# randyjhc/vit-colmap

Measured on AMD Instinct MI355X. Metric: images/sec extracted + pair-matches/sec (N×D brute-force NN), higher is better.
Workload: dtype bf16 (ViT) / u8+i32 (matcher); 1 GPU; configs[1]+configs[2]: DINOv2 ViT-S/14 extract of 50 640x480 images (512 keypoints, 384-D uint8 descriptors) then exhaustive mutual-NN + ratio matching of all pairs among the extracted images; images_total=50, images_rank0=50, num_keypoints=512, descriptor_dim=384, parallelism=images+pairs sharded x1

## Files before the change

### include/vitcolmap_hip.h

```cpp
#ifndef VITCOLMAP_HIP_H_
#define VITCOLMAP_HIP_H_

#include <stddef.h>
#include <stdint.h>

#ifdef __cplusplus
extern "C" {
#endif

#define VC_ABI_VERSION 1

#define VC_OK 0
#define VC_ERR_INVALID_ARG (-1)
#define VC_ERR_UNSUPPORTED (-2)
#define VC_ERR_LAUNCH (-3)
#define VC_ERR_WORKSPACE (-4)

#define VC_MAX_KEYPOINTS 2048
#define VC_MAX_DESC_DIM 1024
#define VC_MAX_NEIGHBOURS 64

typedef void* vc_stream_t;

int vc_abi_version(void);
// ... 134 lines not shown
#define VC_LAYOUT_NCHW 0
#define VC_LAYOUT_PATCHES 1
#define VC_LAYOUT_PATCHES_PAD 2
#define VC_PATCH_K_PADDED 640

int vc_preprocess_u8(const uint8_t* images_bgr, int n_images, int h, int w, int out_h, int out_w,
                     int out_dtype, int layout, void* out, uint8_t* resized_bgr_or_null,
                     vc_stream_t stream);

int vc_add_layernorm_bf16(const void* x, const void* residual_or_null, const void* gamma,
                          const void* beta, float eps, int rows, int C, void* sum_out_or_null,
                          void* y_out, vc_stream_t stream);

int vc_layernorm_drop_first_bf16(const void* x, const void* gamma, const void* beta, float eps, int n_groups,
                                 int group_rows, int C, void* y_out, vc_stream_t stream);

int vc_attention_bf16(const void* qkv, int batch, int n_tokens, int n_heads, int head_dim, int q_prescaled,
                      void* out, vc_stream_t stream);

#define VC_EPI_BIAS 0
#define VC_EPI_GELU 1
#define VC_EPI_RESIDUAL 2
#define VC_EPI_SWIGLU 4
int vc_linear_bf16(const void* x, const void* weight, const void* bias, const void* residual_or_null,
                   void* out, int rows, int n_out, int k_in, int epilogue, vc_stream_t stream);

int vc_conv_taps_bf16(void* x, const void* weight, const void* bias, void* out, int batch, int height, int width, int c_in,
                      int n_out, int kh, int kw, int dy0, int dx0, int out_parity, int epilogue, vc_stream_t stream);

size_t vc_linear_xs_weight_bytes(int n_out, int k_in);
// ... 57 lines not shown
```

### vit_colmap_amd/_lib.py

```python
import ctypes
import os
from ctypes import POINTER, c_char_p, c_double, c_float, c_int, c_int32, c_size_t, c_uint8, c_uint32, c_void_p

_HERE = os.path.dirname(os.path.abspath(__file__))
LIB_PATH = os.environ.get("VITCOLMAP_HIP_LIB") or os.path.join(_HERE, "libvitcolmap_hip.so")

VC_OK = 0
ABI_VERSION = 1
VC_MAX_KEYPOINTS = 2048
VC_MAX_DESC_DIM = 1024
VC_MAX_NEIGHBOURS = 64
VC_BA_MAX_CAMS = 512
VC_BA_MAX_GROUPS = 8
VC_ERR_INVALID_ARG, VC_ERR_UNSUPPORTED, VC_ERR_LAUNCH, VC_ERR_WORKSPACE = -1, -2, -3, -4


class HipLibraryError(RuntimeError):
    pass


_u8p, _i32p, _u32p, _f32p = POINTER(c_uint8), POINTER(c_int32), POINTER(c_uint32), POINTER(ctypes.c_float)

SIGNATURES = {
    "vc_abi_version": (c_int, []),
# ... 42 lines not shown
    "vc_score_map": (c_int, [c_void_p, c_int, c_int, c_int, c_int, c_void_p, c_void_p]),
    "vc_select_keypoints": (c_int, [c_void_p, c_int, c_int, c_int, c_int, c_int, c_float, c_int, c_void_p,
                                    c_void_p, c_void_p, c_void_p, c_void_p, c_void_p, c_void_p]),
    "vc_describe": (c_int, [c_void_p, c_int, c_int, c_int, c_int, c_int, c_void_p, c_void_p, c_int, c_void_p,
                            c_int, c_int, c_int, c_int, c_int, c_void_p, c_void_p, c_void_p, c_void_p]),
    "vc_describe_at": (c_int, [c_void_p, c_int, c_int, c_int, c_int, c_int, c_void_p, c_void_p, c_int, c_void_p, c_int, c_int,
                               c_int, c_int, c_int, c_int, c_void_p, c_void_p, c_void_p]),
    "vc_quantize_u8": (c_int, [c_void_p, c_void_p, c_size_t, c_void_p]),
    "vc_heatmap_workspace_bytes": (c_size_t, [c_int, c_int, c_int, c_int]),
    "vc_heatmap_keypoints": (c_int, [c_void_p, c_void_p, ctypes.c_longlong, ctypes.c_longlong, ctypes.c_longlong, c_int, c_int,
                                     c_int, c_int, c_int, c_float, c_int, c_float, c_float, c_float, c_float, c_void_p,
                                     c_void_p, c_void_p, c_void_p, c_void_p]),
    "vc_add_layernorm_bf16": (c_int, [c_void_p, c_void_p, c_void_p, c_void_p, c_float, c_int, c_int, c_void_p,
                                      c_void_p, c_void_p]),
    "vc_layernorm_drop_first_bf16": (c_int, [c_void_p, c_void_p, c_void_p, c_float, c_int, c_int, c_int, c_void_p, c_void_p]),
    "vc_attention_bf16": (c_int, [c_void_p, c_int, c_int, c_int, c_int, c_int, c_void_p, c_void_p]),
    "vc_linear_bf16": (c_int, [c_void_p, c_void_p, c_void_p, c_void_p, c_void_p, c_int, c_int, c_int, c_int, c_void_p]),
    "vc_conv_taps_bf16": (c_int, [c_void_p, c_void_p, c_void_p, c_void_p] + [c_int] * 11 + [c_void_p]),
    "vc_linear_xs_weight_bytes": (c_size_t, [c_int, c_int]),
    "vc_linear_xs_prepare": (c_int, [c_void_p, c_void_p, c_void_p, c_void_p, c_int, c_int, c_void_p, c_void_p, c_void_p]),
    "vc_linear_xs_bf16": (c_int, [c_void_p, c_void_p, c_void_p, c_void_p, c_void_p, c_int, c_int, c_int, c_int, c_int,
                                  c_float, c_void_p, c_void_p]),
    "vc_gelu_table_bytes": (c_size_t, []),
    "vc_gelu_table_bf16": (c_int, [c_void_p, c_void_p]),
    "vc_patch_embed_bf16": (c_int, [c_void_p, c_void_p, c_void_p, c_void_p, c_void_p, c_int, c_int, c_int, c_int, c_void_p]),
    "vc_mlp_weight_bytes": (c_size_t, [c_int, c_int]),
    "vc_mlp_prepare": (c_int, [c_void_p, c_void_p, c_void_p, c_void_p, c_void_p, c_void_p, c_int, c_int, c_void_p, c_void_p,
                               c_void_p, c_void_p]),
    "vc_mlp_bf16": (c_int, [c_void_p, c_void_p, c_void_p, c_void_p, c_void_p, c_int, c_int, c_int, c_float, c_void_p]),
    "vc_preprocess_u8": (c_int, [c_void_p, c_int, c_int, c_int, c_int, c_int, c_int, c_int, c_void_p, c_void_p,
# ... 102 lines not shown
```

### vit_colmap_amd/csrc/select.hip

```cpp
#include <hip/hip_runtime.h>
#include <stdint.h>

#include "../../include/vitcolmap_hip.h"
#include "common.h"
#include "device.h"

namespace {

constexpr int kMaxCells = 16384;
constexpr int kMaxCandidates = 4096;
constexpr int kSelThreads = 512;

template <typename T>
__device__ inline float load_token(const T* p, int i);
template <>
__device__ inline float load_token<float>(const float* p, int i) { return p[i]; }
template <>
__device__ inline float load_token<uint16_t>(const uint16_t* p, int i) { return vc::bf16_to_f32(p[i]); }

__device__ inline float wave_sum(float v) {
#pragma unroll
  for (int o = 32; o > 0; o >>= 1) v += __shfl_xor(v, o);
  return v;
}

template <typename T>
__global__ __launch_bounds__(256) void structure_tensor_kernel(const T* __restrict__ tokens, int H, int W, int C,
                                                               float* __restrict__ st, bool vec_ok) {
  const int lane = threadIdx.x & 63;
  const int cells = H * W;
  const int cell = blockIdx.x * 4 + (threadIdx.x >> 6);
  const int img = blockIdx.y;
  if (cell >= cells) return;
  const int y = cell / W, x = cell - y * W;
  const T* f = tokens + ((size_t)img * cells + cell) * C;
  const bool has_r = x + 1 < W, has_d = y + 1 < H;
  const T* fr = f + C;
  const T* fd = f + (size_t)W * C;
  float sxx = 0.f, syy = 0.f, sxy = 0.f, sm = 0.f;
  if (vec_ok) {
    typedef uint32_t v4u __attribute__((ext_vector_type(4)));
    constexpr int NQ = (int)sizeof(T) / 2;
    for (int c0 = lane * 8; c0 < C; c0 += 64 * 8) {
      const v4u zero = {0u, 0u, 0u, 0u};
      v4u qv[NQ], qr[NQ], qd[NQ];
#pragma unroll
      for (int q = 0; q < NQ; ++q) {
        qv[q] = *((const v4u*)(f + c0) + q);
        qr[q] = has_r ? *((const v4u*)(fr + c0) + q) : zero;
        qd[q] = has_d ? *((const v4u*)(fd + c0) + q) : zero;
      }
#pragma unroll
      for (int j = 0; j < 8; ++j) {
        float v, r, d;
        if (sizeof(T) == 4) {
          v = __uint_as_float(qv[j >> 2][j & 3]); r = __uint_as_float(qr[j >> 2][j & 3]); d = __uint_as_float(qd[j >> 2][j & 3]);
        } else {
          const int sh = (j & 1) * 16;
          v = __uint_as_float(((qv[0][j >> 1] >> sh) & 0xffffu) << 16);
          r = __uint_as_float(((qr[0][j >> 1] >> sh) & 0xffffu) << 16);
          d = __uint_as_float(((qd[0][j >> 1] >> sh) & 0xffffu) << 16);
        }
        const float gx = has_r ? r - v : 0.f;
        const float gy = has_d ? d - v : 0.f;
        sxx += gx * gx;
        syy += gy * gy;
        sxy += gx * gy;
        sm += v;
      }
    }
  } else {
    for (int c = lane; c < C; c += 64) {
      const float v = load_token<T>(f, c);
      const float gx = has_r ? load_token<T>(fr, c) - v : 0.f;
      const float gy = has_d ? load_token<T>(fd, c) - v : 0.f;
      sxx += gx * gx;
      syy += gy * gy;
      sxy += gx * gy;
      sm += v;
    }
  }
  sxx = wave_sum(sxx); syy = wave_sum(syy); sxy = wave_sum(sxy); sm = wave_sum(sm);
  if (lane == 0) {
    float* o = st + (size_t)img * 4 * cells + cell;
    const float inv = (float)C;
    o[0] = sxx / inv;
    o[cells] = syy / inv;
    o[2 * cells] = sxy / inv;
    o[3 * cells] = sm / inv;
  }
}

struct Taps {
  float w[11];
  int k;
};

__device__ inline float zero_pad(const float* m, int H, int W, int y, int x) {
  return (y >= 0 && y < H && x >= 0 && x < W) ? m[y * W + x] : 0.f;
}

__device__ inline float smooth(const float* m, int H, int W, int y, int x, const Taps& t) {
  const int r = t.k / 2;
  float acc = 0.f;
  for (int dy = 0; dy < t.k; ++dy)
// ... 90 lines not shown

__device__ inline bool before(float sa, int pa, float sb, int pb) { return sa > sb || (sa == sb && pa < pb); }

__global__ __launch_bounds__(kSelThreads) void select_kernel(const float* __restrict__ score_g, int H, int W,
                                                             int target, int bin, int nms_reach, int nms_d2_max, int kmax,
                                                             int32_t* __restrict__ out_yx,
                                                             float* __restrict__ out_score,
                                                             int32_t* __restrict__ out_count,
                                                             int32_t* __restrict__ dbg_cand_yx,
                                                             float* __restrict__ dbg_cand_score,
                                                             int32_t* __restrict__ dbg_cand_count) {
  extern __shared__ __attribute__((aligned(16))) float lds[];
  const int cells = H * W;
  const int tid = threadIdx.x, nt = blockDim.x;
  const int img = blockIdx.x;
  float* score = lds;
  int* cand_cell = (int*)(lds + cells);
  float* cand_score = (float*)(cand_cell + kMaxCandidates);
  int* tmp_cell = (int*)(cand_score + kMaxCandidates);
  float* tmp_score = (float*)(tmp_cell + kMaxCandidates);
  int* state = (int*)(tmp_score + kMaxCandidates);
  int* cell_rank = state + kMaxCandidates;
  __shared__ int s_wave_tot[kSelThreads / 64];

  for (int i = tid; i < cells; i += nt) score[i] = score_g[(size_t)img * cells + i];
  __syncthreads();

  const int nbh = max(1, H / bin), nbw = max(1, W / bin);
  const int per_bin = max(1, target / (nbh * nbw));
  const int bh = min(bin, H), bw = min(bin, W), n = bh * bw;
  const int k = min(per_bin, n);
  const int K_bins = nbh * nbw * k;
  for (int idx = tid; idx < nbh * nbw * n; idx += nt) {
    const int b = idx / n, e = idx - b * n;
    const int bi = b / nbw, bj = b - bi * nbw;
    const int y0 = bi * bin, x0 = bj * bin;
    const int ey = e / bw, ex = e - ey * bw;
    const float s = score[(y0 + ey) * W + x0 + ex];
    int rank = 0;
    for (int oy = 0; oy < bh; ++oy)
      for (int ox = 0; ox < bw; ++ox)
        rank += before(score[(y0 + oy) * W + x0 + ox], oy * bw + ox, s, e) ? 1 : 0;
    if (rank < k) {
      cand_cell[b * k + rank] = (y0 + ey) * W + x0 + ex;
      cand_score[b * k + rank] = s;
    }
  }
  int K = K_bins;
  __syncthreads();

  int run_len = k, n_runs = nbh * nbw;
  auto merged_rank = [&](int e) {
    const float s = cand_score[e];
    const int mine = e / run_len;
    int rank = e - mine * run_len;
    for (int q = 0; q < n_runs; ++q) {
      if (q == mine) continue;
      int lo = 0, hi = run_len;
      while (lo < hi) {
// ... 334 lines not shown
```

### vit_colmap_amd/csrc/vit_ops.hip

```cpp
#include <hip/hip_runtime.h>
#include <stdint.h>

#include "../../include/vitcolmap_hip.h"
#include "common.h"
#include "device.h"

namespace {

typedef uint16_t bf16_t;
constexpr int kMaxChunksPerLane = 4;

__device__ inline float wsum(float v) {
#pragma unroll
  for (int o = 32; o > 0; o >>= 1) v += __shfl_xor(v, o);
  return v;
}

struct alignas(16) Vec8 { bf16_t e[8]; };

template <bool HAS_RES, bool WRITE_SUM>
__global__ __launch_bounds__(256) void add_layernorm_kernel(const bf16_t* __restrict__ x,
                                                            const bf16_t* __restrict__ res,
                                                            const bf16_t* __restrict__ gamma,
                                                            const bf16_t* __restrict__ beta, float eps,
                                                            int rows, int C, bf16_t* __restrict__ sum_out,
                                                            bf16_t* __restrict__ y_out, int drop_group) {
  const int lane = threadIdx.x & 63;
  const int row = blockIdx.x * 4 + (threadIdx.x >> 6);
  if (row >= rows) return;
  const int nchunk = C >> 3;
  const size_t base = (size_t)row * C;
  size_t ybase = base;
  if (drop_group > 0) {
// ... 12 lines not shown
      if (HAS_RES) b = *(const Vec8*)(res + base + ch * 8);
      Vec8 o;
#pragma unroll
      for (int i = 0; i < 8; ++i) {
        float t = vc::bf16_to_f32(a.e[i]);
        if (HAS_RES) {
          o.e[i] = vc::f32_to_bf16(t + vc::bf16_to_f32(b.e[i]));
          t = vc::bf16_to_f32(o.e[i]);
        }
        v[k][i] = t;
        s += t;
      }
      if (HAS_RES && WRITE_SUM) *(Vec8*)(sum_out + base + ch * 8) = o;
    }
  }
  const float mean = wsum(s) / (float)C;
  float q = 0.f;
#pragma unroll
  for (int k = 0; k < kMaxChunksPerLane; ++k) {
    if (lane + 64 * k < nchunk) {
#pragma unroll
      for (int i = 0; i < 8; ++i) { const float d = v[k][i] - mean; q += d * d; }
    }
  }
  const float rstd = rsqrtf(wsum(q) / (float)C + eps);
#pragma unroll
  for (int k = 0; k < kMaxChunksPerLane; ++k) {
    const int ch = lane + 64 * k;
    if (ch < nchunk) {
      const Vec8 g = *(const Vec8*)(gamma + ch * 8);
      const Vec8 bb = *(const Vec8*)(beta + ch * 8);
      Vec8 o;
#pragma unroll
      for (int i = 0; i < 8; ++i) o.e[i] = vc::f32_to_bf16((v[k][i] - mean) * rstd * vc::bf16_to_f32(g.e[i]) + vc::bf16_to_f32(bb.e[i]));
      *(Vec8*)(y_out + ybase + ch * 8) = o;
    }
  }
}

}

extern "C" {

static int add_layernorm_launch(const void* x, const void* residual_or_null, const void* gamma, const void* beta, float eps,
                                int rows, int C, void* sum_out_or_null, void* y_out, int drop_group, vc_stream_t stream);

int vc_add_layernorm_bf16(const void* x, const void* residual_or_null, const void* gamma, const void* beta,
                          float eps, int rows, int C, void* sum_out_or_null, void* y_out, vc_stream_t stream) {
  return add_layernorm_launch(x, residual_or_null, gamma, beta, eps, rows, C, sum_out_or_null, y_out, 0, stream);
}

int vc_layernorm_drop_first_bf16(const void* x, const void* gamma, const void* beta, float eps, int n_groups, int group_rows,
                                 int C, void* y_out, vc_stream_t stream) {
  if (n_groups < 0 || group_rows < 2) return VC_ERR_INVALID_ARG;
  return add_layernorm_launch(x, nullptr, gamma, beta, eps, n_groups * group_rows, C, nullptr, y_out, group_rows, stream);
}

static int add_layernorm_launch(const void* x, const void* residual_or_null, const void* gamma, const void* beta, float eps,
                                int rows, int C, void* sum_out_or_null, void* y_out, int drop_group, vc_stream_t stream) {
  if (!x || !gamma || !beta || !y_out || rows < 0 || C <= 0) return VC_ERR_INVALID_ARG;
  if (C % 8 != 0 || C > 64 * kMaxChunksPerLane * 8) return VC_ERR_UNSUPPORTED;
  if ((((uintptr_t)x) | ((uintptr_t)y_out) | ((uintptr_t)gamma) | ((uintptr_t)beta) |
       ((uintptr_t)residual_or_null) | ((uintptr_t)sum_out_or_null)) % 16 != 0)
    return VC_ERR_INVALID_ARG;
  if (rows == 0) return VC_OK;
  const dim3 grid((rows + 3) / 4), block(256);
  hipStream_t s = (hipStream_t)stream;
  const bf16_t *px = (const bf16_t*)x, *pr = (const bf16_t*)residual_or_null, *pg = (const bf16_t*)gamma,
               *pb = (const bf16_t*)beta;
  bf16_t *ps = (bf16_t*)sum_out_or_null, *py = (bf16_t*)y_out;
  if (!pr)
    hipLaunchKernelGGL((add_layernorm_kernel<false, false>), grid, block, 0, s, px, pr, pg, pb, eps, rows, C, ps, py, drop_group);
  else if (ps)
    hipLaunchKernelGGL((add_layernorm_kernel<true, true>), grid, block, 0, s, px, pr, pg, pb, eps, rows, C, ps, py, drop_group);
  else
    hipLaunchKernelGGL((add_layernorm_kernel<true, false>), grid, block, 0, s, px, pr, pg, pb, eps, rows, C, ps, py, drop_group);
  return vc::check_launch();
}

// ... 2 lines not shown
```

### vit_colmap_amd/features/hip_select.py

```python
import torch

from .. import _lib

METHODS = {"harris": 0, "dog": 1, "combined": 2}


def _dtype_code(t):
    if t.dtype == torch.float32:
        return 0
    if t.dtype == torch.bfloat16:
        return 1
    raise _lib.HipLibraryError(f"tokens must be float32 or bfloat16, got {t.dtype}")


def _check_tokens(tokens, H, W):
    if not tokens.is_cuda:
        raise _lib.HipLibraryError("tokens must live on the GPU (no CPU fallback)")
    assert tokens.dim() == 3 and tokens.is_contiguous() and tokens.shape[1] == H * W, tokens.shape


def structure_tensor(tokens: torch.Tensor, H: int, W: int) -> torch.Tensor:
    _check_tokens(tokens, H, W)
    lib = _lib.load()
    B, _, C = tokens.shape
# ... 75 lines not shown
                                  _lib.ptr(projection), dd, int(feature_wh[0]), int(feature_wh[1]), int(original_wh[0]),
                                  int(original_wh[1]), 1 if rootsift else 0, _lib.ptr(f32), _lib.ptr(u8), _lib.stream_ptr()),
               "vc_describe_at")
    return (u8, f32) if want_f32 else u8


def quantize_u8(x: torch.Tensor) -> torch.Tensor:
    assert x.is_cuda and x.dtype == torch.float32 and x.is_contiguous()
    lib = _lib.load()
    out = torch.empty(x.shape, dtype=torch.uint8, device=x.device)
    _lib.check(lib.vc_quantize_u8(_lib.ptr(x), _lib.ptr(out), x.numel(), _lib.stream_ptr()), "vc_quantize_u8")
    return out


def dense_to_sparse(tokens, H, W, original_wh, resized_wh, num_keypoints, method="harris", projection=None,
                    bin_size=16, nms_radius=1.5, want_f32=False):
    st = structure_tensor(tokens, H, W)
    score = score_map(st, H, W, method)
    yx, sc, cnt = select_keypoints(score, num_keypoints, bin_size, nms_radius)
    out = describe(tokens, H, W, yx, cnt, resized_wh, original_wh, projection, want_f32)
    res = dict(keypoints=out[0], desc_u8=out[1], count=cnt, yx=yx, scores=sc, score=score)
    if want_f32:
        res["desc_f32"] = out[2]
    return res


def heatmap_workspace_bytes(n_images: int, H: int, W: int, kmax: int) -> int:
    return _lib.load().vc_heatmap_workspace_bytes(n_images, H, W, kmax)


def heatmap_keypoints(kp_map: torch.Tensor, desc_map: torch.Tensor, num_keypoints: int, score_threshold: float,
                      nms_radius: int, original_wh, resized_wh):
# ... 24 lines not shown
```

### vit_colmap_amd/features/vit_extractor.py

```python
import os
from pathlib import Path
from typing import Optional

import numpy as np
import torch

from .. import _lib
from ..utils import image_io
from ..vit import build_dinov2, load_dinov2_weights
from . import hip_preprocess, hip_select
from .base_extractor import BaseExtractor, default_camera_params, extract_to_database, host_rows, list_images

PATCH = 14


class ViTExtractor(BaseExtractor):
    camera_params_for = staticmethod(default_camera_params)
    camera_per_image = False

    def __init__(
        self,
        weights_path: str | None = None,
        model_name: str = "dinov2_vitb14",
        num_keypoints: int = 2048,
# ... 79 lines not shown
            files = list_images(Path(image_dir))
            first = image_io.imread(files[0]) if files else None
            if first is not None:
                self._run_batch([first])
        have = vd.broadcast_array(np.array([self.descriptor_projection is not None], np.int32), 0, str(self.device))
        if int(have[0]):
            p = vd.broadcast_array(self.descriptor_projection.cpu().numpy() if rank == 0 else None, 0, str(self.device))
            self.set_projection(p)

    def _require_gpu(self):
        if self.device.type != "cuda":
            raise _lib.HipLibraryError(
                "ViTExtractor needs an MI355X: the selection / descriptor path is HIP-only (no CPU fallback)")

    @torch.inference_mode()
    def _tokens(self, images_bgr: torch.Tensor):
        B, h, w, _ = images_bgr.shape
        hp, wp = h // PATCH, w // PATCH
        if self.model.accepts_padded_patches:
            patches = hip_preprocess.preprocess(images_bgr, out_dtype=self.dtype, layout="patches_pad")
            return self.model.forward_patch_tokens(patches, hp, wp).contiguous(), hp, wp
        patches = hip_preprocess.preprocess(images_bgr, out_dtype=self.dtype, layout="patches")
        if self.tune_gemm:
            import torch.cuda.tunable as tunable

            was = tunable.is_enabled()
            tunable.enable(True)
            try:
                tokens = self.model.forward_patch_tokens(patches, hp, wp).contiguous()
            finally:
                tunable.enable(was)
        else:
            tokens = self.model.forward_patch_tokens(patches, hp, wp).contiguous()
        return tokens, hp, wp

    @torch.inference_mode()
# ... 16 lines not shown
            g = torch.Generator(device="cpu").manual_seed(self.seed)
            p = torch.randn(C, self.descriptor_dim, generator=g, dtype=torch.float32) / np.sqrt(C)
            self.descriptor_projection = p.to(self.device)
            print(f"Initialized random projection (insufficient samples): {C} -> {self.descriptor_dim}")

    batch_shards = None

    def _shard_bounds(self, B, pipelined=False):
        k = self.batch_shards if self.batch_shards is not None else int(os.environ.get("VITCOLMAP_VIT_SHARDS", "1" if pipelined else "2"))
        if k <= 1 or B < 8 * k or not getattr(self.model, "_hip", None):
            return None
        return [B * i // k for i in range(k + 1)]

    def _extract_one(self, images_bgr, hw):
        h, w, h_new, w_new = hw
        tokens, hp, wp = self._tokens(images_bgr)
        self._ensure_projection(tokens, hp, wp, (w, h), (w_new, h_new))
        proj = self.descriptor_projection if tokens.shape[-1] > self.descriptor_dim else None
        return hip_select.dense_to_sparse(tokens, hp, wp, (w, h), (w_new, h_new), self.num_keypoints,
                                          self.detection_method, proj)

    @torch.inference_mode()
    def extract_device(self, images_bgr: torch.Tensor, input_ready=None):
        self._require_gpu()
        B, h, w, _ = images_bgr.shape
        hw = (h, w, (h // PATCH) * PATCH, (w // PATCH) * PATCH)
        bounds = self._shard_bounds(B, pipelined=input_ready is not None)
        needs_fit = self.model.arch.dim > self.descriptor_dim and self.descriptor_projection is None
        if needs_fit or (bounds is None and (input_ready is None or not getattr(self.model, "_hip", None))):
            return self._extract_one(images_bgr, hw)
        if bounds is None:
            bounds = [0, B]
        dev = images_bgr.device
        n_sh = len(bounds) - 1
        n_streams = max(n_sh, int(os.environ.get("VITCOLMAP_VIT_STREAMS", "2")))
# ... 30 lines not shown
            cur.wait_event(done)
            for t in part.values():
                t.record_stream(cur)
        if len(parts) == 1:
            return parts[0]
        return {k: torch.cat([p[k] for p in parts]) for k in parts[0]}

    @torch.inference_mode()
    def _run_batch(self, images_bgr_np):
        self._require_gpu()
        h, w = images_bgr_np[0].shape[:2]
        h_new, w_new = (h // PATCH) * PATCH, (w // PATCH) * PATCH
        if h_new == 0 or w_new == 0:
            raise ValueError(f"image {w}x{h} is smaller than one 14x14 patch")
        batch = torch.from_numpy(np.ascontiguousarray(np.stack(images_bgr_np))).to(self.device, non_blocking=True)
        tokens, hp, wp = self._tokens(batch)
        self._ensure_projection(tokens, hp, wp, (w, h), (w_new, h_new))
        proj = self.descriptor_projection if tokens.shape[-1] > self.descriptor_dim else None
        res = hip_select.dense_to_sparse(tokens, hp, wp, (w, h), (w_new, h_new), self.num_keypoints,
                                         self.detection_method, proj)
        return host_rows(res["count"], res["keypoints"], res["desc_u8"])

    def _staging(self, slot, shape):
        bufs = self.__dict__.setdefault("_pinned_in", {})
        n = int(np.prod(shape))
        if slot not in bufs or bufs[slot].numel() < n:
            bufs[slot] = torch.empty(n, dtype=torch.uint8, pin_memory=True)
        return bufs[slot][:n].view(shape)

    @torch.inference_mode()
    def _launch_batch(self, images_bgr_np):
        self._require_gpu()
        h, w = images_bgr_np[0].shape[:2]
        if (h // PATCH) * PATCH == 0 or (w // PATCH) * PATCH == 0:
            raise ValueError(f"image {w}x{h} is smaller than one 14x14 patch")
# ... 43 lines not shown
```

### vit_colmap_amd/vit/dinov2.py

```python
import math
from dataclasses import dataclass

import torch
import torch.nn as nn
import torch.nn.functional as F

PATCH = 14


@dataclass(frozen=True)
class Arch:
    dim: int
    depth: int
    heads: int
    ffn: str = "mlp"
    registers: int = 0
    img_size: int = 518


DINOV2_ARCHS = {
    "dinov2_vits14": Arch(384, 12, 6),
    "dinov2_vitb14": Arch(768, 12, 12),
    "dinov2_vitl14": Arch(1024, 24, 16),
    "dinov2_vitg14": Arch(1536, 40, 24, ffn="swiglu"),
# ... 173 lines not shown
            if self.accepts_padded_patches:
                self._padded_pos(hp, wp, device)
            elif self.pos_embed.device == device:
                self.interpolated_pos_embed(hp, wp)
            if device.type != "cuda":
                return None
            ev = torch.cuda.Event()
            ev.record(torch.cuda.current_stream(device))
            self._pos_cache[key] = ev
        return ev

    @property
    def accepts_padded_patches(self) -> bool:
        return bool(getattr(self, "_hip", None)) and self.register_tokens is None and not self.training

    def forward_patch_tokens(self, patches: torch.Tensor, hp: int, wp: int) -> torch.Tensor:
        B = patches.shape[0]
        if patches.shape[-1] == 640:
            if not (patches.is_cuda and patches.dtype == torch.bfloat16 and self.register_tokens is None and not self.training):
                raise ValueError("padded patches are only accepted by the bf16 GPU path")
            if getattr(self, "_hip", None) is None:
                self.prepare_hip()
            if not self._hip:
                raise ValueError("padded patches need a model that prepare_hip() covers")
            from . import hip_ops as ops

            pos, cls_row = self._padded_pos(hp, wp, patches.device)
            x = torch.empty((B, 1 + hp * wp, self.arch.dim), dtype=torch.bfloat16, device=patches.device)
            ops.patch_embed(patches, self._pe_w, self.patch_embed.proj.bias, pos, x)
            x[:, 0] = cls_row
            return self._blocks_hip(x)
        if patches.is_cuda and patches.dtype == torch.bfloat16 and getattr(self, "_hip", None) and not self.training:
            from . import hip_ops as ops

            x = ops.linear(F.pad(patches, (0, self._pe_w.shape[1] - patches.shape[-1])), self._pe_w, self.patch_embed.proj.bias)
        else:
            x = self.patch_embed.forward_patches(patches)
        x = torch.cat([self.cls_token.expand(B, -1, -1), x], dim=1) + self.interpolated_pos_embed(hp, wp)
        if self.register_tokens is not None:
            x = torch.cat([x[:, :1], self.register_tokens.expand(B, -1, -1), x[:, 1:]], dim=1)
        if x.is_cuda and x.dtype == torch.bfloat16 and all(b.folded for b in self.blocks) and not self.training:
            x = self._blocks_fused(x.contiguous())
        else:
            for blk in self.blocks:
                x = blk(x)
            x = self.norm(x)
# ... 50 lines not shown
    def _run_sharded(self, x, layer_fn, final_fn, out):
        plan = self._shard_plan(x)
        if plan is None:
            for i in range(len(self.blocks)):
                layer_fn(i, x)
            final_fn(x, out)
            return out
        bounds, side = plan
        cur = torch.cuda.current_stream(x.device)
        streams = [cur] + side
        ready = torch.cuda.Event()
        ready.record(cur)
        for s in side:
            s.wait_event(ready)
        xs = [x[bounds[i]:bounds[i + 1]] for i in range(len(streams))]
        outs = [out[bounds[i]:bounds[i + 1]] for i in range(len(streams))]
        for li in range(len(self.blocks)):
            for s, xi in zip(streams, xs):
                with torch.cuda.stream(s):
                    layer_fn(li, xi)
        for s, xi, oi in zip(streams, xs, outs):
            with torch.cuda.stream(s):
                final_fn(xi, oi)
        for s in side:
            done = torch.cuda.Event()
            done.record(s)
            cur.wait_event(done)
        return out

    def _blocks_hip(self, x, drop_cls: bool = True):
        from . import hip_ops as ops

        if self._hip and self._hip[0].get("kind") == "gemm":
            return self._blocks_gemm(x, drop_cls)
        blocks, hip = list(self.blocks), self._hip

        def layer(i, xi):
            blk, hw = blocks[i], hip[i]
            a = ops.attention(hw["qkv"](xi), blk.attn.num_heads, q_prescaled=True)
            hw["proj"](a, ops.EPI_RESIDUAL, residual=xi, out=xi)
            hw["mlp"](xi)

        return self._run_sharded(x, layer, *self._final_norm(x, drop_cls))

    def _final_norm(self, x, drop_cls):
        from . import hip_ops as ops

        B, N, C = x.shape
        if drop_cls:
            out = torch.empty((B, N - 1, C), dtype=torch.bfloat16, device=x.device)
            return (lambda xi, oi: ops.layernorm_drop_first(xi, self.norm.weight, self.norm.bias, self.norm.eps, out=oi)), out
        out = torch.empty_like(x)

        def all_rows(xi, oi):
            _, h = ops.add_layernorm(xi, None, self.norm.weight, self.norm.bias, self.norm.eps)
            oi.copy_(h)

        return all_rows, out

    def _blocks_gemm(self, x, drop_cls: bool = True):
        from . import hip_ops as ops

        blocks, hip = list(self.blocks), self._hip

        def layer(i, xi):
            blk, hw = blocks[i], hip[i]
            _, h = ops.add_layernorm(xi, None, blk.norm1.weight, blk.norm1.bias, blk.norm1.eps)
            a = ops.attention(ops.linear(h, *hw["qkv"]), blk.attn.num_heads, q_prescaled=True)
            ops.linear(a, *hw["proj"], ops.EPI_RESIDUAL, residual=xi, out=xi)
            _, h = ops.add_layernorm(xi, None, blk.norm2.weight, blk.norm2.bias, blk.norm2.eps)
            if "w12" in hw:
                hdn = ops.linear(h, *hw["w12"], ops.EPI_SWIGLU)
                ops.linear(hdn, *hw["w3"], ops.EPI_RESIDUAL, residual=xi, out=xi)
                return
            hdn = ops.linear(h, *hw["fc1"], ops.EPI_GELU)
            ops.linear(hdn, *hw["fc2"], ops.EPI_RESIDUAL, residual=xi, out=xi)

        return self._run_sharded(x, layer, *self._final_norm(x, drop_cls))

    def _blocks_fused(self, x):
        from .hip_ops import add_layernorm

        if getattr(self, "_hip", None) is None:
            self.prepare_hip()
        if self._hip:
            return self._blocks_hip(x, drop_cls=False)
        blocks = list(self.blocks)
        _, h = add_layernorm(x, None, blocks[0].norm1.weight, blocks[0].norm1.bias, 1e-6)
        for i, blk in enumerate(blocks):
            a = blk.attn(h)
            x, h = add_layernorm(a, x, blk.norm2.weight, blk.norm2.bias, 1e-6)
            m = blk.mlp(h)
            last = i + 1 == len(blocks)
# ... 46 lines not shown
```

### vit_colmap_amd/vit/hip_ops.py

```python
import torch

from .. import _lib


def add_layernorm(x: torch.Tensor, residual, weight: torch.Tensor, bias: torch.Tensor, eps: float,
                  want_sum: bool = True):
    assert x.is_cuda and x.dtype == torch.bfloat16 and x.is_contiguous()
    lib = _lib.load()
    C = x.shape[-1]
    rows = x.numel() // C
    y = torch.empty_like(x)
    s = torch.empty_like(x) if (residual is not None and want_sum) else None
    if residual is not None:
        assert residual.shape == x.shape and residual.dtype == x.dtype and residual.is_contiguous()
    _lib.check(lib.vc_add_layernorm_bf16(_lib.ptr(x), _lib.ptr(residual), _lib.ptr(weight), _lib.ptr(bias), eps, rows, C,
                                         _lib.ptr(s), _lib.ptr(y), _lib.stream_ptr()), "vc_add_layernorm_bf16")
    return s, y


def layernorm_drop_first(x: torch.Tensor, weight: torch.Tensor, bias: torch.Tensor, eps: float, out=None) -> torch.Tensor:
    assert x.is_cuda and x.dtype == torch.bfloat16 and x.is_contiguous() and x.dim() == 3
    B, N, C = x.shape
    y = torch.empty((B, N - 1, C), dtype=torch.bfloat16, device=x.device) if out is None else out
    assert y.shape == (B, N - 1, C) and y.dtype == torch.bfloat16 and y.is_contiguous()
    _lib.check(_lib.load().vc_layernorm_drop_first_bf16(_lib.ptr(x), _lib.ptr(weight), _lib.ptr(bias), eps, B, N, C, _lib.ptr(y),
                                                        _lib.stream_ptr()), "vc_layernorm_drop_first_bf16")
    return y


Q_PRESCALE = 0.125 * 1.4426950408889634


def attention(qkv: torch.Tensor, n_heads: int, q_prescaled: bool = False) -> torch.Tensor:
    assert qkv.is_cuda and qkv.dtype == torch.bfloat16 and qkv.is_contiguous()
    B, N, C3 = qkv.shape
    hd = C3 // (3 * n_heads)
    lib = _lib.load()
    out = torch.empty((B, N, C3 // 3), dtype=torch.bfloat16, device=qkv.device)
    _lib.check(lib.vc_attention_bf16(_lib.ptr(qkv), B, N, n_heads, hd, int(q_prescaled), _lib.ptr(out), _lib.stream_ptr()),
               "vc_attention_bf16")
    return out

# ... 150 lines not shown
```

Measured before the change: 7714 images/s.

## Fuse final layernorm with structure tensor and speed up bin ranking in select

```diff
diff --git a/include/vitcolmap_hip.h b/include/vitcolmap_hip.h
--- a/include/vitcolmap_hip.h
+++ b/include/vitcolmap_hip.h
@@ -172,6 +172,9 @@
 
 int vc_layernorm_drop_first_bf16(const void* x, const void* gamma, const void* beta, float eps, int n_groups,
                                  int group_rows, int C, void* y_out, vc_stream_t stream);
+
+int vc_layernorm_structure_bf16(const void* x, const void* gamma, const void* beta, float eps, int n_groups, int H, int W,
+                                int C, void* y_out, float* st, vc_stream_t stream);
 
 int vc_attention_bf16(const void* qkv, int batch, int n_tokens, int n_heads, int head_dim, int q_prescaled,
                       void* out, vc_stream_t stream);
diff --git a/vit_colmap_amd/_lib.py b/vit_colmap_amd/_lib.py
--- a/vit_colmap_amd/_lib.py
+++ b/vit_colmap_amd/_lib.py
@@ -80,6 +80,8 @@
     "vc_add_layernorm_bf16": (c_int, [c_void_p, c_void_p, c_void_p, c_void_p, c_float, c_int, c_int, c_void_p,
                                       c_void_p, c_void_p]),
     "vc_layernorm_drop_first_bf16": (c_int, [c_void_p, c_void_p, c_void_p, c_float, c_int, c_int, c_int, c_void_p, c_void_p]),
+    "vc_layernorm_structure_bf16": (c_int, [c_void_p, c_void_p, c_void_p, c_float, c_int, c_int, c_int, c_int, c_void_p, c_void_p,
+                                            c_void_p]),
     "vc_attention_bf16": (c_int, [c_void_p, c_int, c_int, c_int, c_int, c_int, c_void_p, c_void_p]),
     "vc_linear_bf16": (c_int, [c_void_p, c_void_p, c_void_p, c_void_p, c_void_p, c_int, c_int, c_int, c_int, c_void_p]),
     "vc_conv_taps_bf16": (c_int, [c_void_p, c_void_p, c_void_p, c_void_p] + [c_int] * 11 + [c_void_p]),
diff --git a/vit_colmap_amd/csrc/select.hip b/vit_colmap_amd/csrc/select.hip
--- a/vit_colmap_amd/csrc/select.hip
+++ b/vit_colmap_amd/csrc/select.hip
@@ -4,6 +4,7 @@
 #include "../../include/vitcolmap_hip.h"
 #include "common.h"
 #include "device.h"
+#include "token_rows.h"
 
 namespace {
 
@@ -18,11 +19,7 @@
 template <>
 __device__ inline float load_token<uint16_t>(const uint16_t* p, int i) { return vc::bf16_to_f32(p[i]); }
 
-__device__ inline float wave_sum(float v) {
-#pragma unroll
-  for (int o = 32; o > 0; o >>= 1) v += __shfl_xor(v, o);
-  return v;
-}
+using vc::wave_sum;
 
 template <typename T>
 __global__ __launch_bounds__(256) void structure_tensor_kernel(const T* __restrict__ tokens, int H, int W, int C,
@@ -37,7 +34,7 @@
   const bool has_r = x + 1 < W, has_d = y + 1 < H;
   const T* fr = f + C;
   const T* fd = f + (size_t)W * C;
-  float sxx = 0.f, syy = 0.f, sxy = 0.f, sm = 0.f;
+  vc::StSums sums;
   if (vec_ok) {
     typedef uint32_t v4u __attribute__((ext_vector_type(4)));
     constexpr int NQ = (int)sizeof(T) / 2;
@@ -61,34 +58,14 @@
           r = __uint_as_float(((qr[0][j >> 1] >> sh) & 0xffffu) << 16);
           d = __uint_as_float(((qd[0][j >> 1] >> sh) & 0xffffu) << 16);
         }
-        const float gx = has_r ? r - v : 0.f;
-        const float gy = has_d ? d - v : 0.f;
-        sxx += gx * gx;
-        syy += gy * gy;
-        sxy += gx * gy;
-        sm += v;
+        sums.add(v, r, d, has_r, has_d);
       }
     }
   } else {
-    for (int c = lane; c < C; c += 64) {
-      const float v = load_token<T>(f, c);
-      const float gx = has_r ? load_token<T>(fr, c) - v : 0.f;
-      const float gy = has_d ? load_token<T>(fd, c) - v : 0.f;
-      sxx += gx * gx;
-      syy += gy * gy;
-      sxy += gx * gy;
-      sm += v;
-    }
-  }
-  sxx = wave_sum(sxx); syy = wave_sum(syy); sxy = wave_sum(sxy); sm = wave_sum(sm);
-  if (lane == 0) {
-    float* o = st + (size_t)img * 4 * cells + cell;
-    const float inv = (float)C;
-    o[0] = sxx / inv;
-    o[cells] = syy / inv;
-    o[2 * cells] = sxy / inv;
-    o[3 * cells] = sm / inv;
-  }
+    for (int c = lane; c < C; c += 64)
+      sums.add(load_token<T>(f, c), has_r ? load_token<T>(fr, c) : 0.f, has_d ? load_token<T>(fd, c) : 0.f, has_r, has_d);
+  }
+  sums.store(lane, st + (size_t)img * 4 * cells + cell, cells, C);
 }
 
 struct Taps {
@@ -209,13 +186,14 @@
   const int cells = H * W;
   const int tid = threadIdx.x, nt = blockDim.x;
   const int img = blockIdx.x;
-  float* score = lds;
-  int* cand_cell = (int*)(lds + cells);
+  int* cand_cell = (int*)lds;
   float* cand_score = (float*)(cand_cell + kMaxCandidates);
   int* tmp_cell = (int*)(cand_score + kMaxCandidates);
   float* tmp_score = (float*)(tmp_cell + kMaxCandidates);
   int* state = (int*)(tmp_score + kMaxCandidates);
   int* cell_rank = state + kMaxCandidates;
+  float* by_bin = (float*)cell_rank;
+  float* score = (float*)(cell_rank + cells);
   __shared__ int s_wave_tot[kSelThreads / 64];
 
   for (int i = tid; i < cells; i += nt) score[i] = score_g[(size_t)img * cells + i];
@@ -226,18 +204,31 @@
   const int bh = min(bin, H), bw = min(bin, W), n = bh * bw;
   const int k = min(per_bin, n);
   const int K_bins = nbh * nbw * k;
+  auto bin_cell = [&](int b, int e) {
+    const int bi = b / nbw, bj = b - bi * nbw;
+    const int ey = e / bw, ex = e - ey * bw;
+    return (bi * bin + ey) * W + bj * bin + ex;
+  };
+  for (int idx = tid; idx < nbh * nbw * n; idx += nt) by_bin[idx] = score[bin_cell(idx / n, idx % n)];
+  __syncthreads();
   for (int idx = tid; idx < nbh * nbw * n; idx += nt) {
     const int b = idx / n, e = idx - b * n;
-    const int bi = b / nbw, bj = b - bi * nbw;
-    const int y0 = bi * bin, x0 = bj * bin;
-    const int ey = e / bw, ex = e - ey * bw;
-    const float s = score[(y0 + ey) * W + x0 + ex];
-    int rank = 0;
-    for (int oy = 0; oy < bh; ++oy)
-      for (int ox = 0; ox < bw; ++ox)
-        rank += before(score[(y0 + oy) * W + x0 + ox], oy * bw + ox, s, e) ? 1 : 0;
+    const float* mine = by_bin + b * n;
+    const float s = mine[e];
+    int rank = 0, same = 0;
+    if (n % 4 == 0) {
+      for (int o = 0; o < n; o += 4) {
+        const float4 q = *(const float4*)(mine + o);
+        rank += (q.x > s ? 1 : 0) + (q.y > s ? 1 : 0) + (q.z > s ? 1 : 0) + (q.w > s ? 1 : 0);
+        same += (q.x == s ? 1 : 0) + (q.y == s ? 1 : 0) + (q.z == s ? 1 : 0) + (q.w == s ? 1 : 0);
+      }
+    } else {
+      for (int o = 0; o < n; ++o) { rank += mine[o] > s ? 1 : 0; same += mine[o] == s ? 1 : 0; }
+    }
+    if (same > 1)
+      for (int o = 0; o < e; ++o) rank += mine[o] == s ? 1 : 0;
     if (rank < k) {
-      cand_cell[b * k + rank] = (y0 + ey) * W + x0 + ex;
+      cand_cell[b * k + rank] = bin_cell(b, e);
       cand_score[b * k + rank] = s;
     }
   }
diff --git a/vit_colmap_amd/csrc/token_rows.h b/vit_colmap_amd/csrc/token_rows.h
--- /dev/null
+++ b/vit_colmap_amd/csrc/token_rows.h
@@ -0,0 +1,63 @@
+#pragma once
+#include <hip/hip_runtime.h>
+#include <stdint.h>
+
+#include "device.h"
+
+namespace vc {
+
+constexpr int kMaxChunksPerLane = 4;
+
+struct alignas(16) Vec8 { uint16_t e[8]; };
+
+__device__ inline float wave_sum(float v) {
+#pragma unroll
+  for (int o = 32; o > 0; o >>= 1) v += __shfl_xor(v, o);
+  return v;
+}
+
+template <int NK>
+__device__ inline void ln_stats(const float (&v)[NK][8], float s, int lane, int nchunk, int C, float eps,
+                                float& mean, float& rstd) {
+  mean = wave_sum(s) / (float)C;
+  float q = 0.f;
+#pragma unroll
+  for (int k = 0; k < NK; ++k) {
+    if (lane + 64 * k < nchunk) {
+#pragma unroll
+      for (int i = 0; i < 8; ++i) { const float d = v[k][i] - mean; q += d * d; }
+    }
+  }
+  rstd = rsqrtf(wave_sum(q) / (float)C + eps);
+}
+
+__device__ inline Vec8 ln_apply(const float (&v)[8], float mean, float rstd, const Vec8& g, const Vec8& b) {
+  Vec8 o;
+#pragma unroll
+  for (int i = 0; i < 8; ++i) o.e[i] = f32_to_bf16((v[i] - mean) * rstd * bf16_to_f32(g.e[i]) + bf16_to_f32(b.e[i]));
+  return o;
+}
+
+struct StSums {
+  float sxx = 0.f, syy = 0.f, sxy = 0.f, sm = 0.f;
+  __device__ inline void add(float v, float r, float d, bool has_r, bool has_d) {
+    const float gx = has_r ? r - v : 0.f;
+    const float gy = has_d ? d - v : 0.f;
+    sxx += gx * gx;
+    syy += gy * gy;
+    sxy += gx * gy;
+    sm += v;
+  }
+  __device__ inline void store(int lane, float* o, int cells, int C) {
+    sxx = wave_sum(sxx); syy = wave_sum(syy); sxy = wave_sum(sxy); sm = wave_sum(sm);
+    if (lane == 0) {
+      const float inv = (float)C;
+      o[0] = sxx / inv;
+      o[cells] = syy / inv;
+      o[2 * cells] = sxy / inv;
+      o[3 * cells] = sm / inv;
+    }
+  }
+};
+
+}
diff --git a/vit_colmap_amd/csrc/vit_ops.hip b/vit_colmap_amd/csrc/vit_ops.hip
--- a/vit_colmap_amd/csrc/vit_ops.hip
+++ b/vit_colmap_amd/csrc/vit_ops.hip
@@ -4,19 +4,13 @@
 #include "../../include/vitcolmap_hip.h"
 #include "common.h"
 #include "device.h"
+#include "token_rows.h"
 
 namespace {
 
 typedef uint16_t bf16_t;
-constexpr int kMaxChunksPerLane = 4;
-
-__device__ inline float wsum(float v) {
-#pragma unroll
-  for (int o = 32; o > 0; o >>= 1) v += __shfl_xor(v, o);
-  return v;
-}
-
-struct alignas(16) Vec8 { bf16_t e[8]; };
+using vc::kMaxChunksPerLane;
+using vc::Vec8;
 
 template <bool HAS_RES, bool WRITE_SUM>
 __global__ __launch_bounds__(256) void add_layernorm_kernel(const bf16_t* __restrict__ x,
@@ -59,28 +53,68 @@
       if (HAS_RES && WRITE_SUM) *(Vec8*)(sum_out + base + ch * 8) = o;
     }
   }
-  const float mean = wsum(s) / (float)C;
-  float q = 0.f;
-#pragma unroll
-  for (int k = 0; k < kMaxChunksPerLane; ++k) {
-    if (lane + 64 * k < nchunk) {
-#pragma unroll
-      for (int i = 0; i < 8; ++i) { const float d = v[k][i] - mean; q += d * d; }
-    }
-  }
-  const float rstd = rsqrtf(wsum(q) / (float)C + eps);
+  float mean, rstd;
+  vc::ln_stats(v, s, lane, nchunk, C, eps, mean, rstd);
 #pragma unroll
   for (int k = 0; k < kMaxChunksPerLane; ++k) {
     const int ch = lane + 64 * k;
+    if (ch < nchunk)
+      *(Vec8*)(y_out + ybase + ch * 8) = vc::ln_apply(v[k], mean, rstd, *(const Vec8*)(gamma + ch * 8), *(const Vec8*)(beta + ch * 8));
+  }
+}
+
+template <int NK>
+__global__ __launch_bounds__(256) void layernorm_structure_kernel(const bf16_t* __restrict__ x,
+                                                                  const bf16_t* __restrict__ gamma,
+                                                                  const bf16_t* __restrict__ beta, float eps, int H, int W,
+                                                                  int C, bf16_t* __restrict__ y_out, float* __restrict__ st) {
+  const int lane = threadIdx.x & 63;
+  const int cells = H * W;
+  const int cell = blockIdx.x * 4 + (threadIdx.x >> 6);
+  const int img = blockIdx.y;
+  if (cell >= cells) return;
+  const int cy = cell / W, cx = cell - cy * W;
+  const bool has[3] = {true, cx + 1 < W, cy + 1 < H};
+  const int nchunk = C >> 3;
+  const bf16_t* row0 = x + ((size_t)img * (cells + 1) + 1 + cell) * C;
+  const bf16_t* rows[3] = {row0, row0 + C, row0 + (size_t)W * C};
+  float v[3][NK][8];
+  float mean[3], rstd[3];
+#pragma unroll
+  for (int t = 0; t < 3; ++t) {
+    float s = 0.f;
+#pragma unroll
+    for (int k = 0; k < NK; ++k) {
+      const int ch = lane + 64 * k;
+      if (ch < nchunk && has[t]) {
+        const Vec8 a = *(const Vec8*)(rows[t] + ch * 8);
+#pragma unroll
+        for (int i = 0; i < 8; ++i) {
+          v[t][k][i] = vc::bf16_to_f32(a.e[i]);
+          s += v[t][k][i];
+        }
+      }
+    }
+    vc::ln_stats(v[t], s, lane, has[t] ? nchunk : 0, C, eps, mean[t], rstd[t]);
+  }
+  vc::StSums sums;
+#pragma unroll
+  for (int k = 0; k < NK; ++k) {
+    const int ch = lane + 64 * k;
     if (ch < nchunk) {
       const Vec8 g = *(const Vec8*)(gamma + ch * 8);
-      const Vec8 bb = *(const Vec8*)(beta + ch * 8);
-      Vec8 o;
+      const Vec8 b = *(const Vec8*)(beta + ch * 8);
+      Vec8 o[3] = {};
 #pragma unroll
-      for (int i = 0; i < 8; ++i) o.e[i] = vc::f32_to_bf16((v[k][i] - mean) * rstd * vc::bf16_to_f32(g.e[i]) + vc::bf16_to_f32(bb.e[i]));
-      *(Vec8*)(y_out + ybase + ch * 8) = o;
+      for (int t = 0; t < 3; ++t)
+        if (has[t]) o[t] = vc::ln_apply(v[t][k], mean[t], rstd[t], g, b);
+      *(Vec8*)(y_out + ((size_t)img * cells + cell) * C + ch * 8) = o[0];
+#pragma unroll
+      for (int i = 0; i < 8; ++i)
+        sums.add(vc::bf16_to_f32(o[0].e[i]), vc::bf16_to_f32(o[1].e[i]), vc::bf16_to_f32(o[2].e[i]), has[1], has[2]);
     }
   }
+  sums.store(lane, st + (size_t)img * 4 * cells + cell, cells, C);
 }
 
 }
@@ -101,13 +135,32 @@
   return add_layernorm_launch(x, nullptr, gamma, beta, eps, n_groups * group_rows, C, nullptr, y_out, group_rows, stream);
 }
 
-static int add_layernorm_launch(const void* x, const void* residual_or_null, const void* gamma, const void* beta, float eps,
-                                int rows, int C, void* sum_out_or_null, void* y_out, int drop_group, vc_stream_t stream) {
+static int layernorm_args(const void* x, const void* residual_or_null, const void* gamma, const void* beta, int rows, int C,
+                          void* sum_out_or_null, void* y_out) {
   if (!x || !gamma || !beta || !y_out || rows < 0 || C <= 0) return VC_ERR_INVALID_ARG;
   if (C % 8 != 0 || C > 64 * kMaxChunksPerLane * 8) return VC_ERR_UNSUPPORTED;
   if ((((uintptr_t)x) | ((uintptr_t)y_out) | ((uintptr_t)gamma) | ((uintptr_t)beta) |
        ((uintptr_t)residual_or_null) | ((uintptr_t)sum_out_or_null)) % 16 != 0)
     return VC_ERR_INVALID_ARG;
+  return VC_OK;
+}
+
+int vc_layernorm_structure_bf16(const void* x, const void* gamma, const void* beta, float eps, int n_groups, int H, int W, int C,
+                                void* y_out, float* st, vc_stream_t stream) {
+  if (n_groups < 0 || H <= 0 || W <= 0 || !st) return VC_ERR_INVALID_ARG;
+  if (n_groups > 65535 || ((long)H * W + 1) * (n_groups > 0 ? n_groups : 1) > 0x7fffffffL) return VC_ERR_UNSUPPORTED;
+  if (int rc = layernorm_args(x, nullptr, gamma, beta, n_groups * (H * W + 1), C, nullptr, y_out)) return rc;
+  if (n_groups == 0) return VC_OK;
+  return vc::dispatch<1, 2, 3, 4>((C + 511) / 512, [&](auto nk) {
+    hipLaunchKernelGGL(layernorm_structure_kernel<nk.value>, dim3((H * W + 3) / 4, n_groups), dim3(256), 0, (hipStream_t)stream,
+                       (const bf16_t*)x, (const bf16_t*)gamma, (const bf16_t*)beta, eps, H, W, C, (bf16_t*)y_out, st);
+    return vc::check_launch();
+  });
+}
+
+static int add_layernorm_launch(const void* x, const void* residual_or_null, const void* gamma, const void* beta, float eps,
+                                int rows, int C, void* sum_out_or_null, void* y_out, int drop_group, vc_stream_t stream) {
+  if (int rc = layernorm_args(x, residual_or_null, gamma, beta, rows, C, sum_out_or_null, y_out)) return rc;
   if (rows == 0) return VC_OK;
   const dim3 grid((rows + 3) / 4), block(256);
   hipStream_t s = (hipStream_t)stream;
diff --git a/vit_colmap_amd/features/hip_select.py b/vit_colmap_amd/features/hip_select.py
--- a/vit_colmap_amd/features/hip_select.py
+++ b/vit_colmap_amd/features/hip_select.py
@@ -113,8 +113,9 @@
 
 
 def dense_to_sparse(tokens, H, W, original_wh, resized_wh, num_keypoints, method="harris", projection=None,
-                    bin_size=16, nms_radius=1.5, want_f32=False):
-    st = structure_tensor(tokens, H, W)
+                    bin_size=16, nms_radius=1.5, want_f32=False, st=None):
+    if st is None:
+        st = structure_tensor(tokens, H, W)
     score = score_map(st, H, W, method)
     yx, sc, cnt = select_keypoints(score, num_keypoints, bin_size, nms_radius)
     out = describe(tokens, H, W, yx, cnt, resized_wh, original_wh, projection, want_f32)
diff --git a/vit_colmap_amd/features/vit_extractor.py b/vit_colmap_amd/features/vit_extractor.py
--- a/vit_colmap_amd/features/vit_extractor.py
+++ b/vit_colmap_amd/features/vit_extractor.py
@@ -117,12 +117,17 @@
                 "ViTExtractor needs an MI355X: the selection / descriptor path is HIP-only (no CPU fallback)")
 
     @torch.inference_mode()
-    def _tokens(self, images_bgr: torch.Tensor):
+    def _tokens(self, images_bgr: torch.Tensor, want_st: bool = False):
         B, h, w, _ = images_bgr.shape
         hp, wp = h // PATCH, w // PATCH
         if self.model.accepts_padded_patches:
             patches = hip_preprocess.preprocess(images_bgr, out_dtype=self.dtype, layout="patches_pad")
+            if want_st:
+                tokens, st = self.model.forward_patch_tokens(patches, hp, wp, want_st=True)
+                return tokens.contiguous(), hp, wp, st
             return self.model.forward_patch_tokens(patches, hp, wp).contiguous(), hp, wp
+        if want_st:
+            return self._tokens(images_bgr) + (None,)
         patches = hip_preprocess.preprocess(images_bgr, out_dtype=self.dtype, layout="patches")
         if self.tune_gemm:
             import torch.cuda.tunable as tunable
@@ -169,11 +174,11 @@
 
     def _extract_one(self, images_bgr, hw):
         h, w, h_new, w_new = hw
-        tokens, hp, wp = self._tokens(images_bgr)
+        tokens, hp, wp, st = self._tokens(images_bgr, want_st=True)
         self._ensure_projection(tokens, hp, wp, (w, h), (w_new, h_new))
         proj = self.descriptor_projection if tokens.shape[-1] > self.descriptor_dim else None
         return hip_select.dense_to_sparse(tokens, hp, wp, (w, h), (w_new, h_new), self.num_keypoints,
-                                          self.detection_method, proj)
+                                          self.detection_method, proj, st=st)
 
     @torch.inference_mode()
     def extract_device(self, images_bgr: torch.Tensor, input_ready=None):
@@ -234,11 +239,11 @@
         if h_new == 0 or w_new == 0:
             raise ValueError(f"image {w}x{h} is smaller than one 14x14 patch")
         batch = torch.from_numpy(np.ascontiguousarray(np.stack(images_bgr_np))).to(self.device, non_blocking=True)
-        tokens, hp, wp = self._tokens(batch)
+        tokens, hp, wp, st = self._tokens(batch, want_st=True)
         self._ensure_projection(tokens, hp, wp, (w, h), (w_new, h_new))
         proj = self.descriptor_projection if tokens.shape[-1] > self.descriptor_dim else None
         res = hip_select.dense_to_sparse(tokens, hp, wp, (w, h), (w_new, h_new), self.num_keypoints,
-                                         self.detection_method, proj)
+                                         self.detection_method, proj, st=st)
         return host_rows(res["count"], res["keypoints"], res["desc_u8"])
 
     def _staging(self, slot, shape):
diff --git a/vit_colmap_amd/vit/dinov2.py b/vit_colmap_amd/vit/dinov2.py
--- a/vit_colmap_amd/vit/dinov2.py
+++ b/vit_colmap_amd/vit/dinov2.py
@@ -211,7 +211,14 @@
     def accepts_padded_patches(self) -> bool:
         return bool(getattr(self, "_hip", None)) and self.register_tokens is None and not self.training
 
-    def forward_patch_tokens(self, patches: torch.Tensor, hp: int, wp: int) -> torch.Tensor:
+    def forward_patch_tokens(self, patches: torch.Tensor, hp: int, wp: int, want_st: bool = False):
+        if want_st:
+            if patches.shape[-1] == 640:
+                return self._forward_patch_tokens(patches, hp, wp, (hp, wp))
+            return self._forward_patch_tokens(patches, hp, wp), None
+        return self._forward_patch_tokens(patches, hp, wp)
+
+    def _forward_patch_tokens(self, patches, hp, wp, st_grid=None):
         B = patches.shape[0]
         if patches.shape[-1] == 640:
             if not (patches.is_cuda and patches.dtype == torch.bfloat16 and self.register_tokens is None and not self.training):
@@ -226,7 +233,7 @@
             x = torch.empty((B, 1 + hp * wp, self.arch.dim), dtype=torch.bfloat16, device=patches.device)
             ops.patch_embed(patches, self._pe_w, self.patch_embed.proj.bias, pos, x)
             x[:, 0] = cls_row
-            return self._blocks_hip(x)
+            return self._blocks_hip(x, st_grid=st_grid)
         if patches.is_cuda and patches.dtype == torch.bfloat16 and getattr(self, "_hip", None) and not self.training:
             from . import hip_ops as ops
 
@@ -307,7 +314,8 @@
         for s in side:
             s.wait_event(ready)
         xs = [x[bounds[i]:bounds[i + 1]] for i in range(len(streams))]
-        outs = [out[bounds[i]:bounds[i + 1]] for i in range(len(streams))]
+        cut = lambda t, i: tuple(u[bounds[i]:bounds[i + 1]] for u in t) if isinstance(t, tuple) else t[bounds[i]:bounds[i + 1]]
+        outs = [cut(out, i) for i in range(len(streams))]
         for li in range(len(self.blocks)):
             for s, xi in zip(streams, xs):
                 with torch.cuda.stream(s):
@@ -321,11 +329,11 @@
             cur.wait_event(done)
         return out
 
-    def _blocks_hip(self, x, drop_cls: bool = True):
+    def _blocks_hip(self, x, drop_cls: bool = True, st_grid=None):
         from . import hip_ops as ops
 
         if self._hip and self._hip[0].get("kind") == "gemm":
-            return self._blocks_gemm(x, drop_cls)
+            return self._blocks_gemm(x, drop_cls, st_grid)
         blocks, hip = list(self.blocks), self._hip
 
         def layer(i, xi):
@@ -334,12 +342,18 @@
             hw["proj"](a, ops.EPI_RESIDUAL, residual=xi, out=xi)
             hw["mlp"](xi)
 
-        return self._run_sharded(x, layer, *self._final_norm(x, drop_cls))
-
-    def _final_norm(self, x, drop_cls):
+        return self._run_sharded(x, layer, *self._final_norm(x, drop_cls, st_grid))
+
+    def _final_norm(self, x, drop_cls, st_grid=None):
         from . import hip_ops as ops
 
         B, N, C = x.shape
+        if drop_cls and st_grid is not None:
+            hp, wp = st_grid
+            out = (torch.empty((B, N - 1, C), dtype=torch.bfloat16, device=x.device),
+                   torch.empty((B, 4, N - 1), dtype=torch.float32, device=x.device))
+            return (lambda xi, oi: ops.layernorm_structure(xi, self.norm.weight, self.norm.bias, self.norm.eps, hp, wp,
+                                                           out=oi[0], st_out=oi[1])), out
         if drop_cls:
             out = torch.empty((B, N - 1, C), dtype=torch.bfloat16, device=x.device)
             return (lambda xi, oi: ops.layernorm_drop_first(xi, self.norm.weight, self.norm.bias, self.norm.eps, out=oi)), out
@@ -351,7 +365,7 @@
 
         return all_rows, out
 
-    def _blocks_gemm(self, x, drop_cls: bool = True):
+    def _blocks_gemm(self, x, drop_cls: bool = True, st_grid=None):
         from . import hip_ops as ops
 
         blocks, hip = list(self.blocks), self._hip
@@ -369,7 +383,7 @@
             hdn = ops.linear(h, *hw["fc1"], ops.EPI_GELU)
             ops.linear(hdn, *hw["fc2"], ops.EPI_RESIDUAL, residual=xi, out=xi)
 
-        return self._run_sharded(x, layer, *self._final_norm(x, drop_cls))
+        return self._run_sharded(x, layer, *self._final_norm(x, drop_cls, st_grid))
 
     def _blocks_fused(self, x):
         from .hip_ops import add_layernorm
diff --git a/vit_colmap_amd/vit/hip_ops.py b/vit_colmap_amd/vit/hip_ops.py
--- a/vit_colmap_amd/vit/hip_ops.py
+++ b/vit_colmap_amd/vit/hip_ops.py
@@ -26,6 +26,20 @@
     _lib.check(_lib.load().vc_layernorm_drop_first_bf16(_lib.ptr(x), _lib.ptr(weight), _lib.ptr(bias), eps, B, N, C, _lib.ptr(y),
                                                         _lib.stream_ptr()), "vc_layernorm_drop_first_bf16")
     return y
+
+
+def layernorm_structure(x: torch.Tensor, weight: torch.Tensor, bias: torch.Tensor, eps: float, H: int, W: int, out=None,
+                        st_out=None):
+    assert x.is_cuda and x.dtype == torch.bfloat16 and x.is_contiguous() and x.dim() == 3
+    B, N, C = x.shape
+    assert N == 1 + H * W, (x.shape, H, W)
+    y = torch.empty((B, N - 1, C), dtype=torch.bfloat16, device=x.device) if out is None else out
+    st = torch.empty((B, 4, N - 1), dtype=torch.float32, device=x.device) if st_out is None else st_out
+    assert y.shape == (B, N - 1, C) and y.dtype == torch.bfloat16 and y.is_contiguous()
+    assert st.shape == (B, 4, N - 1) and st.dtype == torch.float32 and st.is_contiguous()
+    _lib.check(_lib.load().vc_layernorm_structure_bf16(_lib.ptr(x), _lib.ptr(weight), _lib.ptr(bias), eps, B, H, W, C, _lib.ptr(y),
+                                                       _lib.ptr(st), _lib.stream_ptr()), "vc_layernorm_structure_bf16")
+    return y, st
 
 
 Q_PRESCALE = 0.125 * 1.4426950408889634
```

Measured after the change: 7741 images/s (median of 6 runs). No clear change (+0.4%).
